# tatsuya-ogawa/metal4-raytracing

Hardware: AMD Instinct MI355X
Metric: Grays/sec (closest-hit + shadow rays traced) at 1920x1080x4spp, dragon; ms/frame (higher is better)
Workload: dtype f32; 1 GPU; c3g: glass dragon scene (configs[2]) 1920x1080x4spp, 8 bounces, one frame per step, single GPU, frames submitted back to back (overlapping frames in flight); scene=c3g, triangles=881218, width=1920, height=1080, spp=4, max_bounces=8, pipeline=wavefront, parallelism=tiles1, rays_per_frame=31537269, sort_bins=0, bvh=sah, frames_in_flight=8, animate=False

## Files before the change

### __graft_entry__.py

```python
import importlib
import lzma
import os
import shutil
import subprocess
import sys

ROOT = os.path.dirname(os.path.abspath(__file__))
PKG = "metal4-raytracing_amd"
ASSET_SRC = os.path.join(ROOT, "tests", "golden", "scene_data")
ASSET_FILES = ["plane.obj", "plane.mtl", "plane-back.obj", "plane-back.mtl", "sphere.obj", "sphere.mtl",
               "dragon.mtl", "train.obj", "train.mtl", "treefir.obj", "treefir.mtl", "teapot.obj",
               "coatball/coatball.obj", "coatball/coatball.mtl"]


def build() -> None:
    env = dict(os.environ, PYTORCH_ROCM_ARCH="gfx950")
    jobs = str(min(16, os.cpu_count() or 1))
    subprocess.run(["make", "-j", jobs, "-C", os.path.join(ROOT, PKG)], check=True, env=env)
    subprocess.run(["make", "-j", jobs, "-C", os.path.join(ROOT, "oracle")], check=True, env=env)
    subprocess.run(["make", "-C", os.path.join(ROOT, "host")], check=True, env=env)
    subprocess.run(["make", "-C", os.path.join(ROOT, "tests", "graph_repro")], check=True, env=env)
    dst = os.path.join(ROOT, "assets")
    for f in ASSET_FILES:
        src, out = os.path.join(ASSET_SRC, f), os.path.join(dst, f)
        if os.path.exists(out):
            continue
        os.makedirs(os.path.dirname(out), exist_ok=True)
        if os.path.exists(src):
            shutil.copyfile(src, out)
        else:
            with lzma.open(src + ".xz", "rb") as fi, open(out + ".tmp", "wb") as fo:
                shutil.copyfileobj(fi, fo)
            os.replace(out + ".tmp", out)
    if ROOT not in sys.path:
        sys.path.insert(0, ROOT)
    rt = importlib.import_module(PKG)
    rt.lib()


def smoke() -> None:
    if ROOT not in sys.path:
        sys.path.insert(0, ROOT)
    import numpy as np
    rt = importlib.import_module(PKG)
    import oracle
    scene = rt.Scene.preset("c1")
    osc = oracle.OracleScene(scene.desc())
    for pipeline in ("wavefront", "megakernel"):
        R = rt.Renderer(scene, 64, 64, device=0, seed=1, pipeline=pipeline)
        R.samplesPerPixel = 1
        R.maxBounces = 2
        u = R.draw()
        g = R.radiance()
        o = osc.render(u, R.random)["radiance"]
        err = np.linalg.norm((g - o)[..., :3], axis=-1) / np.maximum(np.linalg.norm(o[..., :3], axis=-1), 1e-6)
        assert float(err.max()) <= 1e-4, f"smoke parity failed ({pipeline}): max rel L2 {err.max()}"
        print(f"smoke ok ({pipeline}): {rt.version()}, 64x64 c1 frame, max rel L2 {err.max():.3g}, "
              f"bitwise {np.mean(np.all(g[..., :3] == o[..., :3], axis=-1)):.4f}")
        R.close()

if __name__ == "__main__":
    build()
    if len(sys.argv) > 1 and sys.argv[1] == "smoke":
        smoke()
```

### metal4-raytracing_amd/csrc/rt_device.h

```cpp
#pragma once
#include <hip/hip_runtime.h>
#include "rt_math.h"
#include "../../include/rt_types.h"
#include "rt_bvh.h"

namespace rt {

constexpr int kStackSize = 16;
constexpr int kBlock = 256;

struct RootBoxes;
struct DevScene {
    const float* tris;
    const Bvh8Node* nodes8;
    const RootBoxes* root_box;
    const uint4* tri_info;
    const float4* pos;
    const float4* prev_pos;
    const float4* nrm;
    const float4* tri_nrm;
    const float* inst;
    const float* prev_inst;
    const Material* materials;
    const Light* lights;
    const HaltonDim* halton;
    const uint16_t* tri_bin;
    int max_submeshes;
    int num_materials;
    int num_tris;
    int num_nodes8;
    const uchar4* tex_texels = nullptr;
    const uint4* tex_info = nullptr;
    const int4* mat_tex = nullptr;
    const float2* uv = nullptr;
    const float* tex_lut = nullptr;
    int textured = 0;
};

struct Hit {
    float t;
    uint32_t id;
    float u, v;
};

__host__ __device__ __forceinline__ f3 ld3(const float4& v) { return mk3(v.x, v.y, v.z); }

constexpr int kTriFloats = 16;
__host__ __device__ __forceinline__ const float* tri_rec(const float* tris, uint32_t slot) {
    return tris + (size_t)kTriFloats * slot;
}
struct Win3 { float a, b, c; };
__host__ __device__ __forceinline__ f3 tri_window(const float* rec, int v, int kz) {
    const Win3 w = *reinterpret_cast<const Win3*>(rec + 5 * v + kz);
    return mk3(w.a, w.b, w.c);
}
__host__ __device__ __forceinline__ uint32_t tri_id_at(const float* tris, uint32_t fidx) {
    return *reinterpret_cast<const uint32_t*>(reinterpret_cast<const char*>(tris) + fidx * 4u + 60u);
}
__host__ __device__ __forceinline__ f3 tri_window_at(const float* tris, uint32_t fidx) {
    const Win3 w = *reinterpret_cast<const Win3*>(reinterpret_cast<const char*>(tris) + fidx * 4u);
    return mk3(w.a, w.b, w.c);
}
__host__ __device__ __forceinline__ uint32_t tri_id(const float* rec) { return __builtin_bit_cast(uint32_t, rec[15]); }
__host__ __device__ __forceinline__ f3 tri_vertex(const float* rec, int v) { return mk3(rec[5 * v], rec[5 * v + 1], rec[5 * v + 2]); }
__host__ __device__ __forceinline__ void tri_store(float* rec, const float* w, uint32_t id) {
    for (int v = 0; v < 3; ++v) {
        rec[5 * v + 0] = w[3 * v + 0];
        rec[5 * v + 1] = w[3 * v + 1];
        rec[5 * v + 2] = w[3 * v + 2];
        rec[5 * v + 3] = w[3 * v + 0];
        rec[5 * v + 4] = w[3 * v + 1];
    }
    rec[15] = __builtin_bit_cast(float, id);
}

__host__ __device__ __forceinline__ f3 xform(const float* m, f3 p, float w) {
    f3 c0 = mk3(m[0], m[1], m[2]), c1 = mk3(m[3], m[4], m[5]), c2 = mk3(m[6], m[7], m[8]), c3 = mk3(m[9], m[10], m[11]);
    return ((c0 * p.x + c1 * p.y) + c2 * p.z) + c3 * w;
}

struct TraceCounters {
    uint32_t nodes;
    uint32_t tris;
    uint32_t lds_nodes;
};

struct RaySetup {
    f3 o;
    RayPre pre;
    float ix, iy, iz;
    float ox, oy, oz;
    uint32_t dneg;
};

__host__ __device__ __forceinline__ RaySetup ray_setup(f3 o, f3 d) {
    RaySetup R;
    R.pre = ray_precompute(d);
    R.o = rot3(o, R.pre.kz);
    auto safe_inv = [](float x) {
        x = fabsf(x) < 1e-30f ? copysignf(1e-30f, x) : x;
#if defined(__HIP_DEVICE_COMPILE__)
        return __builtin_amdgcn_rcpf(x);
#else
        return 1.0f / x;
#endif
    };
    R.ix = safe_inv(d.x);
    R.iy = safe_inv(d.y);
    R.iz = safe_inv(d.z);
    R.ox = o.x * R.ix;
    R.oy = o.y * R.iy;
    R.oz = o.z * R.iz;
    R.dneg = (d.x < 0.0f ? 1u : 0u) | (d.y < 0.0f ? 2u : 0u) | (d.z < 0.0f ? 4u : 0u);
    return R;
}

__host__ __device__ __forceinline__ float byte_f(uint32_t w, int b) { return (float)((w >> (8 * b)) & 0xffu); }

struct NodeU3 { uint32_t x, y, z; };
struct NodeWords {
    float4 h0;
    NodeU3 h1;
    uint4 qx, qy, qz;
};
__host__ __device__ __forceinline__ NodeWords load_node8(const Bvh8Node* nodes, uint32_t ni) {
    const char* base = reinterpret_cast<const char*>(nodes);
    const uint32_t o = ni * (uint32_t)sizeof(Bvh8Node);
    NodeWords w;
    w.h0 = *reinterpret_cast<const float4*>(base + o);
    w.h1 = *reinterpret_cast<const NodeU3*>(base + (o + 16u));
    w.qx = *reinterpret_cast<const uint4*>(base + (o + 32u));
    w.qy = *reinterpret_cast<const uint4*>(base + (o + 48u));
    w.qz = *reinterpret_cast<const uint4*>(base + (o + 64u));
    return w;
}

__host__ __device__ __forceinline__ uint32_t spread_nibbles(uint32_t x) {
    x = (x | (x << 12)) & 0x000F000Fu;
    x = (x | (x << 6)) & 0x03030303u;
    x = (x | (x << 3)) & 0x11111111u;
    return x * 15u;
}
__host__ __device__ __forceinline__ uint32_t tri_slot(uint32_t tri_base, uint32_t tri_valid, int k) {
    return tri_base + (uint32_t)__builtin_popcount(tri_valid & ((1u << k) - 1u));
}

__host__ __device__ __forceinline__ uint32_t node8_hit_slots(const NodeWords& W, const RaySetup& R, float tmin, float tmax) {
    const float4 h0 = W.h0;
    const uint4 qx = W.qx, qy = W.qy, qz = W.qz;
    const uint32_t ew = __builtin_bit_cast(uint32_t, h0.w);
    const float sx = __builtin_bit_cast(float, (ew & 0xffu) << 23);
    const float sy = __builtin_bit_cast(float, ((ew >> 8) & 0xffu) << 23);
    const float sz = __builtin_bit_cast(float, ((ew >> 16) & 0xffu) << 23);
    const float ax = sx * R.ix, ay = sy * R.iy, az = sz * R.iz;
    const float bx = __builtin_fmaf(h0.x, R.ix, -R.ox);
    const float by = __builtin_fmaf(h0.y, R.iy, -R.oy);
    const float bz = __builtin_fmaf(h0.z, R.iz, -R.oz);
    const uint32_t nx0 = R.ix >= 0.0f ? qx.x : qx.z, nx1 = R.ix >= 0.0f ? qx.y : qx.w;
    const uint32_t fx0 = R.ix >= 0.0f ? qx.z : qx.x, fx1 = R.ix >= 0.0f ? qx.w : qx.y;
    const uint32_t ny0 = R.iy >= 0.0f ? qy.x : qy.z, ny1 = R.iy >= 0.0f ? qy.y : qy.w;
    const uint32_t fy0 = R.iy >= 0.0f ? qy.z : qy.x, fy1 = R.iy >= 0.0f ? qy.w : qy.y;
    const uint32_t nz0 = R.iz >= 0.0f ? qz.x : qz.z, nz1 = R.iz >= 0.0f ? qz.y : qz.w;
    const uint32_t fz0 = R.iz >= 0.0f ? qz.z : qz.x, fz1 = R.iz >= 0.0f ? qz.w : qz.y;
    const float tf_max = tmax * 1.0000004f;
    uint32_t hm = 0;
    #pragma unroll
    for (int c = 0; c < 8; ++c) {
        const int b = c & 3;
        const uint32_t wnx = c < 4 ? nx0 : nx1, wfx = c < 4 ? fx0 : fx1;
        const uint32_t wny = c < 4 ? ny0 : ny1, wfy = c < 4 ? fy0 : fy1;
        const uint32_t wnz = c < 4 ? nz0 : nz1, wfz = c < 4 ? fz0 : fz1;
        const float tnx = __builtin_fmaf(byte_f(wnx, b), ax, bx), tfx = __builtin_fmaf(byte_f(wfx, b), ax, bx);
        const float tny = __builtin_fmaf(byte_f(wny, b), ay, by), tfy = __builtin_fmaf(byte_f(wfy, b), ay, by);
        const float tnz = __builtin_fmaf(byte_f(wnz, b), az, bz), tfz = __builtin_fmaf(byte_f(wfz, b), az, bz);
        const float tn = fmaxf(fmaxf(tnx, tny), fmaxf(tnz, tmin));
        const float tf = fminf(fminf(tfx, tfy), fminf(tfz, tf_max));
        const bool hit = tn <= tf;
        hm |= hit ? (1u << c) : 0u;
    }
    return hm;
}
__host__ __device__ __forceinline__ void node8_decode(uint32_t hm, uint32_t ew, const NodeU3& h1, uint32_t dneg,
                                                      uint32_t& ihits, uint32_t& tmask, uint32_t& tvalid,
                                                      uint32_t& child_base, uint32_t& tri_base, bool& flip) {
    const int axis = (int)((ew >> 24) & 3u);
    const uint32_t k_int = ew >> 28;
    ihits = hm & ((1u << k_int) - 1u);
    tmask = spread_nibbles(hm >> k_int) & h1.z;
    tvalid = h1.z;
    child_base = h1.x;
    tri_base = h1.y;
    flip = (dneg >> axis) & 1u;
}
__host__ __device__ __forceinline__ void test_node8_words(const NodeWords& W, const RaySetup& R, float tmin, float tmax,
                                                          uint32_t& ihits, uint32_t& tmask, uint32_t& tvalid,
                                                          uint32_t& child_base, uint32_t& tri_base, bool& flip) {
    const uint32_t hm = node8_hit_slots(W, R, tmin, tmax);
    node8_decode(hm, __builtin_bit_cast(uint32_t, W.h0.w), W.h1, R.dneg, ihits, tmask, tvalid, child_base, tri_base, flip);
}

#ifndef RT_ROOT_MASK
#define RT_ROOT_MASK 1
#endif
constexpr uint32_t kRootValid = 0x100u;
__host__ __device__ __forceinline__ uint32_t root_word(const NodeWords& root, f3 o, f3 d, float tmax) {
#if RT_ROOT_MASK
    return kRootValid | node8_hit_slots(root, ray_setup(o, d), 0.0f, tmax);
#else
    return 0u;
#endif
}
#ifndef RT_ROOT_TIGHT
#define RT_ROOT_TIGHT 1
#endif
struct RootBoxes {
    float b[3][2][8];
    uint32_t used;
    uint32_t reserved[3];
};
static_assert(sizeof(RootBoxes) == 208, "RootBoxes: 48 planes and the used word, 16-B rows");

__host__ __device__ __forceinline__ bool root_child_bounds(const Bvh8Node* nodes, const float* node_box, const float* tris,
                                                           int c, float lo[3], float hi[3]) {
    const Bvh8Node& nd = nodes[0];
    for (int a = 0; a < 3; ++a) {
        lo[a] = INFINITY;
        hi[a] = -INFINITY;
    }
    if (nd.q[c] == 255 && nd.q[8 + c] == 0) return false;
    const int k_int = nd.axis_k >> 4;
    if (c < k_int) {
        const float* bx = node_box + 6 * (size_t)(nd.child_base + (uint32_t)c);
        for (int a = 0; a < 3; ++a) {
            lo[a] = bx[a];
            hi[a] = bx[3 + a];
        }
    } else {
        const int j = c - k_int;
        const uint32_t first = nd.tri_base + bvh8_leaf_first(nd.tri_valid, j), n = bvh8_leaf_count(nd.tri_valid, j);
        for (uint32_t t = 0; t < n; ++t)
            for (int q = 0; q < 3; ++q) {
                const f3 v = tri_vertex(tri_rec(tris, first + t), q);
                lo[0] = fminf(lo[0], v.x); hi[0] = fmaxf(hi[0], v.x);
                lo[1] = fminf(lo[1], v.y); hi[1] = fmaxf(hi[1], v.y);
                lo[2] = fminf(lo[2], v.z); hi[2] = fmaxf(hi[2], v.z);
            }
        if (n == 0) return false;
    }
    return true;
}
constexpr float kRootPadRel = 1.0f / 524288.0f;
__host__ __device__ __forceinline__ void root_box_store(RootBoxes& B, int c, bool used, const float lo[3], const float hi[3],
                                                        const float pad[3]) {
    for (int a = 0; a < 3; ++a) {
        B.b[a][0][c] = used ? lo[a] - pad[a] : INFINITY;
        B.b[a][1][c] = used ? hi[a] + pad[a] : -INFINITY;
    }
}
__host__ __device__ inline void root_boxes_fill(RootBoxes& B, const Bvh8Node* nodes, const float* node_box, const float* tris) {
    float lo[8][3], hi[8][3], m[3] = {0.0f, 0.0f, 0.0f};
    bool used[8];
    for (int c = 0; c < 8; ++c) {
        used[c] = root_child_bounds(nodes, node_box, tris, c, lo[c], hi[c]);
        for (int a = 0; a < 3; ++a)
            if (used[c]) m[a] = fmaxf(m[a], fmaxf(fabsf(lo[c][a]), fabsf(hi[c][a])));
    }
    const float pad[3] = {kRootPadRel * m[0], kRootPadRel * m[1], kRootPadRel * m[2]};
    B.used = 0u;
// ... 106 lines not shown
```

### metal4-raytracing_amd/csrc/rt_math.h

```cpp
#pragma once

#include <stdint.h>
#include <math.h>

#if defined(__HIPCC__) || defined(__HIP_DEVICE_COMPILE__)
#include <hip/hip_runtime.h>
#define RT_HD __host__ __device__ __forceinline__
#else
#define RT_HD static inline
#endif

#if defined(__clang__)
#pragma clang fp contract(off)
#endif

namespace rt {

struct f3 { float x, y, z; };
struct f2 { float x, y; };

RT_HD f3 mk3(float x, float y, float z) { f3 r; r.x = x; r.y = y; r.z = z; return r; }
RT_HD f3 operator+(f3 a, f3 b) { return mk3(a.x + b.x, a.y + b.y, a.z + b.z); }
RT_HD f3 operator-(f3 a, f3 b) { return mk3(a.x - b.x, a.y - b.y, a.z - b.z); }
RT_HD f3 operator-(f3 a) { return mk3(-a.x, -a.y, -a.z); }
RT_HD f3 operator*(f3 a, f3 b) { return mk3(a.x * b.x, a.y * b.y, a.z * b.z); }
RT_HD f3 operator*(f3 a, float s) { return mk3(a.x * s, a.y * s, a.z * s); }
RT_HD f3 operator*(float s, f3 a) { return mk3(s * a.x, s * a.y, s * a.z); }
RT_HD f3 operator/(f3 a, float s) { return mk3(a.x / s, a.y / s, a.z / s); }
RT_HD float dot(f3 a, f3 b) { return (a.x * b.x + a.y * b.y) + a.z * b.z; }
RT_HD f3 cross(f3 a, f3 b) {
    return mk3(a.y * b.z - a.z * b.y, a.z * b.x - a.x * b.z, a.x * b.y - a.y * b.x);
}
RT_HD float length(f3 a) { return sqrtf(dot(a, a)); }
RT_HD bool length_lt_1e10(f3 a) { return dot(a, a) < 0x1.79ca1p-67f; }
RT_HD bool length_lt_1e3(f3 a) { return dot(a, a) < 0x1.0c6f7ap-20f; }
RT_HD bool length_gt_1e4(f3 a) { return dot(a, a) > 0x1.5798eep-27f; }
RT_HD f3 normalize(f3 a) { float inv = 1.0f / sqrtf(dot(a, a)); return a * inv; }
RT_HD float clampf(float x, float lo, float hi) { return fminf(fmaxf(x, lo), hi); }
RT_HD float saturate(float x) { return clampf(x, 0.0f, 1.0f); }
RT_HD float mixf(float x, float y, float a) { return x + (y - x) * a; }
RT_HD f3 mix3(f3 x, f3 y, float a) { return mk3(mixf(x.x, y.x, a), mixf(x.y, y.y, a), mixf(x.z, y.z, a)); }
RT_HD f3 mix3v(f3 x, f3 y, f3 a) { return mk3(mixf(x.x, y.x, a.x), mixf(x.y, y.y, a.y), mixf(x.z, y.z, a.z)); }

static constexpr float RT_PI = 3.14159265358979323846f;

RT_HD void sincos_pinned(float x, float* s, float* c) {
    float j = rintf(x * 0.63661977236758134f);
    int q = (int)j;
    float r = x - j * 1.5703125f;
    r = r - j * 4.837512969970703125e-4f;
    r = r - j * 7.54978995489188216e-8f;
    float z = r * r;
    float sr = r + r * z * (-1.6666654611e-1f + z * (8.3321608736e-3f + z * (-1.9515295891e-4f)));
    float cr = (1.0f - 0.5f * z) + z * z * (4.166664568298827e-2f + z * (-1.388731625493765e-3f + z * 2.443315711809948e-5f));
    switch (q & 3) {
        case 0: *s = sr; *c = cr; break;
        case 1: *s = cr; *c = -sr; break;
        case 2: *s = -sr; *c = -cr; break;
        default: *s = -cr; *c = sr; break;
    }
}
RT_HD float cos_pinned(float x) { float s, c; sincos_pinned(x, &s, &c); return c; }
RT_HD float pow5(float x) { float x2 = x * x; return (x2 * x2) * x; }

static constexpr int RT_HALTON_DIMS = 1024;
static constexpr int RT_MAX_BOUNCES = 12;

struct HaltonDim { uint32_t b; uint32_t m; uint32_t sh; float invB; };

inline void halton_table_fill(HaltonDim* t, int n) {
    int have = 0;
    for (uint32_t c = 2; have < n; ++c) {
        bool prime = true;
        for (int k = 0; k < have; ++k) {
            if (t[k].b * t[k].b > c) break;
            if (c % t[k].b == 0) { prime = false; break; }
        }
        if (!prime) continue;
        HaltonDim h;
        h.b = c;
        uint32_t l = 0;
        while ((1u << l) < c) ++l;
        h.m = (uint32_t)(((1ull << (31 + l)) + c - 1) / c);
        h.sh = l - 1;
        h.invB = 1.0f / (float)c;
        t[have++] = h;
    }
}

RT_HD uint32_t umulhi32(uint32_t a, uint32_t b) {
#if defined(__HIP_DEVICE_COMPILE__)
    return __umulhi(a, b);
#else
    return (uint32_t)(((uint64_t)a * (uint64_t)b) >> 32);
#endif
}

RT_HD float halton_fast(int i, const HaltonDim& h) {
    float f = 1.0f, r = 0.0f;
    uint32_t n = (uint32_t)i;
    if (i <= 0) return 0.0f;
    while (n > 0) {
        f = f * h.invB;
        uint32_t q = umulhi32(n, h.m) >> h.sh;
        r = r + f * (float)(n - q * h.b);
        n = q;
    }
    return r;
}

RT_HD uint32_t bitrev32(uint32_t x) {
#if defined(__HIP_DEVICE_COMPILE__)
    return __builtin_bitreverse32(x);
#else
    x = ((x >> 1) & 0x55555555u) | ((x & 0x55555555u) << 1);
    x = ((x >> 2) & 0x33333333u) | ((x & 0x33333333u) << 2);
    x = ((x >> 4) & 0x0f0f0f0fu) | ((x & 0x0f0f0f0fu) << 4);
    x = ((x >> 8) & 0x00ff00ffu) | ((x & 0x00ff00ffu) << 8);
    return (x >> 16) | (x << 16);
#endif
}
RT_HD float halton_base2(int i) {
    if (i <= 0) return 0.0f;
    const uint32_t b = bitrev32((uint32_t)i);
    uint32_t r = b;
    const int drop = 8 - __builtin_clz(b);
    if (drop > 0) {
        const uint32_t half = (b >> (drop - 1)) & 1u, last = (b >> drop) & 1u;
        r = b & ~((1u << drop) - 1u);
        if (half & last) {
            r += 1u << drop;
            if (r == 0u) return 1.0f;
        }
    }
    return (float)r * 2.3283064365386963e-10f;
}

RT_HD f3 sampleCosineWeightedHemisphere(float ux, float uy) {
    float phi = 2.0f * RT_PI * ux;
    float sin_phi, cos_phi;
    sincos_pinned(phi, &sin_phi, &cos_phi);
    float cos_theta = sqrtf(uy);
    float sin_theta = sqrtf(1.0f - cos_theta * cos_theta);
    return mk3(sin_theta * cos_phi, cos_theta, sin_theta * sin_phi);
}
RT_HD f3 alignHemisphereWithNormal(f3 s, f3 normal) {
    f3 up = normal;
    f3 right = normalize(cross(normal, mk3(0.0072f, 1.0f, 0.0034f)));
    f3 forward = cross(right, up);
    return (s.x * right + s.y * up) + s.z * forward;
}
RT_HD float distributionGGX(float NdotH, float alpha) {
    float a2 = alpha * alpha;
    float denom = (NdotH * NdotH) * (a2 - 1.0f) + 1.0f;
    return a2 / fmaxf(RT_PI * denom * denom, 1e-7f);
}
RT_HD float geometrySchlickGGX(float NdotV, float k) {
    return NdotV / fmaxf(NdotV * (1.0f - k) + k, 1e-7f);
}
RT_HD float geometrySmith(float NdotV, float NdotL, float k) {
    return geometrySchlickGGX(NdotV, k) * geometrySchlickGGX(NdotL, k);
}
RT_HD f3 fresnelSchlick(float cosTheta, f3 F0) {
    float p = pow5(clampf(1.0f - cosTheta, 0.0f, 1.0f));
    return mk3(F0.x + (1.0f - F0.x) * p, F0.y + (1.0f - F0.y) * p, F0.z + (1.0f - F0.z) * p);
}

struct RayPre {
    int kz;
    float Sx, Sy, Sz;
};
RT_HD float comp(f3 v, int k) { return k == 0 ? v.x : (k == 1 ? v.y : v.z); }
RT_HD f3 rot3(f3 v, int kz) { return kz == 0 ? mk3(v.x, v.y, v.z) : (kz == 1 ? mk3(v.y, v.z, v.x) : mk3(v.z, v.x, v.y)); }
RT_HD RayPre ray_precompute(f3 d) {
    RayPre p;
    float ax = fabsf(d.x), ay = fabsf(d.y), az = fabsf(d.z);
    int kz = (ax > ay) ? ((ax > az) ? 0 : 2) : ((ay > az) ? 1 : 2);
    const f3 r = rot3(d, kz);
    p.kz = kz;
    p.Sx = r.y / r.x;
    p.Sy = r.z / r.x;
    p.Sz = 1.0f / r.x;
    return p;
}
RT_HD bool intersect_rot(const RayPre& p, f3 o, f3 a, f3 b, f3 c, float tmin, float tmax,
                         float* t_out, float* V_out, float* W_out, float* det_out) {
    const float Akz = a.x - o.x, Bkz = b.x - o.x, Ckz = c.x - o.x;
    const float Ax = (a.y - o.y) - p.Sx * Akz;
    const float Ay = (a.z - o.z) - p.Sy * Akz;
    const float Bx = (b.y - o.y) - p.Sx * Bkz;
    const float By = (b.z - o.z) - p.Sy * Bkz;
    const float Cx = (c.y - o.y) - p.Sx * Ckz;
    const float Cy = (c.z - o.z) - p.Sy * Ckz;
    float U = Cx * By - Cy * Bx;
    float V = Ax * Cy - Ay * Cx;
    float W = Bx * Ay - By * Ax;
    if ((U < 0.0f || V < 0.0f || W < 0.0f) && (U > 0.0f || V > 0.0f || W > 0.0f)) return false;
    float det = (U + V) + W;
    if (det == 0.0f) return false;
    float Az = p.Sz * Akz, Bz = p.Sz * Bkz, Cz = p.Sz * Ckz;
    float T = (U * Az + V * Bz) + W * Cz;
    float t = T / det;
    if (!(t >= tmin && t <= tmax)) return false;
    *t_out = t;
    *V_out = V;
    *W_out = W;
    *det_out = det;
    return true;
}
RT_HD bool intersect_triangle_vw(const RayPre& p, f3 o, f3 v0, f3 v1, f3 v2, float tmin, float tmax,
                                 float* t_out, float* V_out, float* W_out, float* det_out) {
    return intersect_rot(p, rot3(o, p.kz), rot3(v0, p.kz), rot3(v1, p.kz), rot3(v2, p.kz), tmin, tmax, t_out, V_out,
                         W_out, det_out);
}

}
```

### metal4-raytracing_amd/csrc/rt_trav.h

```cpp
#pragma once
#include "rt_device.h"

namespace rt {

struct Trav {
    RaySetup R;
    float best, bu, bv, bdet;
    uint32_t best_id, g_base, g_hits, t_base, t_mask, t_valid;
    bool g_flip, hit_any;
    int sp;
};

__host__ __device__ __forceinline__ void trav_start(Trav& T, f3 o, f3 d, float tmax) {
    T.R = ray_setup(o, d);
    T.best = tmax;
    T.best_id = 0xffffffffu;
    T.bu = T.bv = 0.0f;
    T.bdet = 1.0f;
    T.g_base = 0;
    T.g_hits = 1;
    T.g_flip = false;
    T.t_mask = 0;
    T.sp = 0;
    T.hit_any = false;
}

__host__ __device__ __forceinline__ bool trav_start_root(Trav& T, f3 o, f3 d, float tmax, uint32_t word, const RootHead& H) {
    trav_start(T, o, d, tmax);
    if (!(word & kRootValid)) return false;
    node8_decode(word & 0xffu, H.ew, H.h1, T.R.dneg, T.g_hits, T.t_mask, T.t_valid, T.g_base, T.t_base, T.g_flip);
    return true;
}

__host__ __device__ __forceinline__ uint32_t next_node(Trav& T, int* stack, bool& overflow) {
    if (!T.g_hits) {
        --T.sp;
        const uint32_t ent = (uint32_t)stack[T.sp * kBlock];
        unpack_group(ent, T.g_base, T.g_flip, T.g_hits);
    }
    const int r = T.g_flip ? highest_bit(T.g_hits) : lowest_bit(T.g_hits);
    T.g_hits &= ~(1u << r);
    if (T.g_hits) {
        if (T.sp < kStackSize) {
            stack[T.sp * kBlock] = (int)pack_group(T.g_base, T.g_flip, T.g_hits);
            ++T.sp;
        } else {
            overflow = true;
        }
    }
    return T.g_base + (uint32_t)r;
}

template <bool COUNT>
__host__ __device__ __forceinline__ void node_step(const DevScene& S, Trav& T, int* stack, TraceCounters& tc, bool& overflow,
                                                   float cull) {
    const uint32_t ni = next_node(T, stack, overflow);
    if (COUNT) tc.nodes++;
    const NodeWords w = load_node8(S.nodes8, ni);
    test_node8_words(w, T.R, 0.0f, fminf(cull, T.best), T.g_hits, T.t_mask, T.t_valid, T.g_base, T.t_base, T.g_flip);
}

template <bool COUNT>
__host__ __device__ __forceinline__ bool trav_step(const DevScene& S, Trav& T, bool any, int* stack, TraceCounters& tc,
                                                   bool& overflow, float cull) {
    bool tdone = false;
    if (T.t_mask != 0u) {
        const int k0 = lowest_bit(T.t_mask);
        T.t_mask &= T.t_mask - 1u;
        const bool two = T.t_mask != 0u;
        const int k1 = two ? lowest_bit(T.t_mask) : k0;
        if (two) T.t_mask &= T.t_mask - 1u;
        const uint32_t kz = (uint32_t)T.R.pre.kz;
        const uint32_t f0 = tri_slot(T.t_base, T.t_valid, k0) * (uint32_t)kTriFloats + kz;
        const uint32_t f1 = tri_slot(T.t_base, T.t_valid, k1) * (uint32_t)kTriFloats + kz;
        const f3 a0 = tri_window_at(S.tris, f0), a1 = tri_window_at(S.tris, f0 + 5u), a2 = tri_window_at(S.tris, f0 + 10u);
        const uint32_t ida = tri_id_at(S.tris, f0 - kz);
        const f3 b0 = tri_window_at(S.tris, f1), b1 = tri_window_at(S.tris, f1 + 5u), b2 = tri_window_at(S.tris, f1 + 10u);
        const uint32_t idb = tri_id_at(S.tris, f1 - kz);
        if (COUNT) tc.tris += two ? 2u : 1u;
        auto accept = [&](float t, float u, float v, float dt, uint32_t id) {
            if (any) {
                T.hit_any = true;
                tdone = true;
            } else if (t < T.best || id < T.best_id) {
                T.best = t;
                T.best_id = id;
                T.bu = u;
                T.bdet = dt;
                T.bv = v;
            }
        };
        float t, u, v, dt;
        if (intersect_rot(T.R.pre, T.R.o, a0, a1, a2, 0.0f, fminf(cull, T.best), &t, &u, &v, &dt)) accept(t, u, v, dt, ida);
        if (two && !tdone && intersect_rot(T.R.pre, T.R.o, b0, b1, b2, 0.0f, fminf(cull, T.best), &t, &u, &v, &dt))
            accept(t, u, v, dt, idb);
    }
    if (!tdone && T.t_mask == 0u && (T.g_hits != 0u || T.sp > 0)) node_step<COUNT>(S, T, stack, tc, overflow, cull);
    return tdone || (T.t_mask == 0u && T.g_hits == 0u && T.sp == 0);
}

}
```

### metal4-raytracing_amd/csrc/rt_wavefront.hip

```cpp
#include "rt_shade.h"
#include "rt_trav.h"
#include "rt_wavefront.h"
#include "rt_wf_queue.h"

#include <array>
#include <utility>

namespace rt {

namespace {

constexpr uint32_t kNoKey = 0xffffffffu;

__device__ __forceinline__ void ts_start(const WfParams& Q, int ts) {
    if (ts >= 0 && blockIdx.x == 0 && threadIdx.x == 0) Q.W.tstamp[ts * kTsStride] = __builtin_amdgcn_s_memrealtime();
}
__device__ __forceinline__ void ts_end(const WfParams& Q, int ts, uint32_t* done) {
    if (ts < 0 || lane_id() != 0) return;
    if (atomicAdd(done, 1u) == (blockDim.x + 63u) / 64u - 1u)
        atomicMax(&Q.W.tstamp[ts * kTsStride + kTsLine * (1 + (int)(blockIdx.x % (uint32_t)kTsXcds))],
                  (unsigned long long)__builtin_amdgcn_s_memrealtime());
}

__device__ __forceinline__ void stat_add(const WfParams& Q, int word, uint32_t v) {
// ... 285 lines not shown
            h.id = __float_as_uint(hv.y);
            h.u = hv.z;
            h.v = hv.w;
            pid = __float_as_uint(o.w);
            if (!SORTED || h.id != 0xffffffffu) {
                uint4 meta;
                PathRegs p;
                load_path(P, Q, o, d, [&]() { return SORTED ? Q.W.sorted[ce] : ld_stream(&Q.W.qc[cur][ce]); }, FULL, pid,
                          meta, p);
                const f3 a = p.accum;
                int sample = (int)meta.y;
                rayO = ld3(o);
                rayD = ld3(d);
                shade_step<FULL, false>(S, U, halton, (int)meta.w, sample, rayO, rayD, h, p, sample == 0 && p.step == 0,
                                 zero2, false, zero2, r);
                write_pixel_outputs(P, meta.x, r, h, FULL);
                nstate = pack_state(p.bounce, p.tpass, p.step);
                front = likely_long(p);
                ncol = make_float4(p.color.x, p.color.y, p.color.z, __uint_as_float(meta.w));
                if (__float_as_uint(p.accum.x) != __float_as_uint(a.x) || __float_as_uint(p.accum.y) != __float_as_uint(a.y) ||
                    __float_as_uint(p.accum.z) != __float_as_uint(a.z)) {
                    if (!FULL) {
                        const float4 s = Q.W.p_accum[pid];
                        p.accum = mk3(s.x + p.accum.x, s.y + p.accum.y, s.z + p.accum.z);
                    }
                    Q.W.p_accum[pid] = make_float4(p.accum.x, p.accum.y, p.accum.z, 0.0f);
                }
            }
        }
        const uint32_t rwn = r.next ? producer_root_word(lds_root, rayO, rayD, INFINITY) : 0u;
        const bool dead = r.next && root_retires(rwn);
        n_retired += (uint32_t)__popcll(__ballot(dead));
        r.next = r.next && !dead;
        const bool pr[3] = {r.shadow, r.next && front, r.next && !front};
        uint32_t* const ctr[3] = {&Q.W.counts[cslot(kCntShadowQ + shard)], &Q.W.counts[cslot(next * kShards + shard)],
                                  &Q.W.counts[cslot(kCntBack + next * kShards + shard)]};
        uint32_t slots[3];
        const uint32_t oct = (rayD.x < 0.0f ? 1u : 0u) | (rayD.y < 0.0f ? 2u : 0u) | (rayD.z < 0.0f ? 4u : 0u);
        block_alloc3_oct(pr, oct, ctr, bao, slots);
        const uint32_t ns = slots[0], nr = front ? slots[1] : Q.seg_cap - 1u - slots[2];
        if (r.shadow) {
            sqout[3 * (size_t)ns] = make_float4(r.so.x, r.so.y, r.so.z, __uint_as_float(pid));
            sqout[3 * (size_t)ns + 1] = make_float4(r.sd.x, r.sd.y, r.sd.z, r.stmax);
            sqout[3 * (size_t)ns + 2] = make_float4(r.contrib.x, r.contrib.y, r.contrib.z,
                                                    __uint_as_float(producer_root_word(lds_root, r.so, r.sd, r.stmax)));
        }
        if (r.next) {
            qout[2 * (size_t)nr] = make_float4(rayO.x, rayO.y, rayO.z, __uint_as_float(pid));
            qout[2 * (size_t)nr + 1] = make_float4(rayD.x, rayD.y, rayD.z, __uint_as_float(nstate));
            qcout[nr] = ncol;
            qrout[nr] = rwn;
        }
    }
    flush_producer(P, Q, n_retired, 0);
}

__device__ __forceinline__ void sort_range(uint32_t n, uint32_t& beg, uint32_t& end) {
    beg = (uint32_t)(((uint64_t)n * blockIdx.x) / kSortBlocks);
    end = (uint32_t)(((uint64_t)n * (blockIdx.x + 1)) / kSortBlocks);
}

__device__ __forceinline__ uint32_t sort_key(const DevScene& S, const WfParams& Q, uint32_t e, uint32_t shift) {
    const uint32_t id = __float_as_uint(Q.W.hits[e].y);
    return id == 0xffffffffu ? kNoKey : ((uint32_t)S.tri_bin[id] >> shift);
}

__global__ void __launch_bounds__(kSortThreads) wf_sort_hist(DevScene S, WfParams Q, int cur) {
    __shared__ uint32_t h[kSortMaxBins];
    if (tail_mode(Q)) return;
    const uint32_t shift = __builtin_ctz(kSortMaxBins) - __builtin_ctz(Q.sort_bins);
    const uint32_t K = Q.sort_bins;
    const QueueShards qs = load_queue(Q.W.counts, cur, Q.seg_cap);
    for (uint32_t k = threadIdx.x; k < K; k += kSortThreads) h[k] = 0;
    __syncthreads();
    uint32_t beg, end;
    sort_range(queue_len(qs), beg, end);
    for (uint32_t g = beg + threadIdx.x; g < end; g += kSortThreads) {
        const uint32_t k = sort_key(S, Q, dense_entry(qs, g, Q.seg_cap), shift);
        if (k != kNoKey) atomicAdd(&h[k], 1u);
    }
    __syncthreads();
    for (uint32_t k = threadIdx.x; k < K; k += kSortThreads) Q.W.sort_table[(size_t)k * kSortBlocks + blockIdx.x] = h[k];
}

__global__ void __launch_bounds__(kSortBlocks) wf_sort_rowscan(WfParams Q) {
    __shared__ uint32_t w[kSortBlocks / 64];
    if (tail_mode(Q)) return;
    uint32_t* row = Q.W.sort_table + (size_t)blockIdx.x * kSortBlocks;
    const uint32_t v = row[threadIdx.x];
    const uint32_t incl = wave_incl_scan(v);
    uint32_t base, total;
    block_prefix<kSortBlocks / 64>(lane_id() == 63, incl, w, base, total);
    row[threadIdx.x] = base + incl - v;
    if (threadIdx.x == kSortBlocks - 1) Q.W.sort_total[blockIdx.x] = total;
}

__global__ void __launch_bounds__(kSortThreads) wf_sort_scatter(DevScene S, WfParams Q, int cur) {
    __shared__ uint32_t off[kSortMaxBins];
    if (tail_mode(Q)) return;
    const uint32_t shift = __builtin_ctz(kSortMaxBins) - __builtin_ctz(Q.sort_bins);
    __shared__ uint32_t w[kSortThreads / 64];
    const uint32_t K = Q.sort_bins, per = K / kSortThreads;
    const QueueShards qs = load_queue(Q.W.counts, cur, Q.seg_cap);
    uint32_t loc[kSortMaxBins / kSortThreads];
    uint32_t s = 0;
    for (uint32_t i = 0; i < per; ++i) {
        loc[i] = s;
        s += Q.W.sort_total[threadIdx.x * per + i];
    }
    const uint32_t incl = wave_incl_scan(s);
    uint32_t base, total;
    block_prefix<kSortThreads / 64>(lane_id() == 63, incl, w, base, total);
    const uint32_t excl = base + incl - s;
    for (uint32_t i = 0; i < per; ++i) {
        const uint32_t k = threadIdx.x * per + i;
        off[k] = excl + loc[i] + Q.W.sort_table[(size_t)k * kSortBlocks + blockIdx.x];
    }
    if (blockIdx.x == 0 && threadIdx.x == kSortThreads - 1) Q.W.counts[cslot(kCntSorted)] = total;
    __syncthreads();
    const float4* qin = Q.W.q[cur];
    uint32_t beg, end;
    sort_range(queue_len(qs), beg, end);
    for (uint32_t g = beg + threadIdx.x; g < end; g += kSortThreads) {
        const uint32_t e = dense_entry(qs, g, Q.seg_cap);
        const float4 hv = Q.W.hits[e];
        const uint32_t id = __float_as_uint(hv.y);
        if (id == 0xffffffffu) continue;
        const uint32_t pos = atomicAdd(&off[(uint32_t)S.tri_bin[id] >> shift], 1u);
        const float4 o = qin[2 * (size_t)e], d = qin[2 * (size_t)e + 1];
        Q.W.sorted[4 * (size_t)pos] = o;
        Q.W.sorted[4 * (size_t)pos + 1] = d;
        Q.W.sorted[4 * (size_t)pos + 2] = hv;
        if (__float_as_uint(d.w) != 0u) Q.W.sorted[4 * (size_t)pos + 3] = Q.W.qc[cur][e];
    }
}

__device__ __forceinline__ void connect_flush(const WfParams& Q, const float4* qin, uint32_t* pend, uint32_t& npend) {
    __builtin_amdgcn_fence(__ATOMIC_SEQ_CST, "wavefront");
    __builtin_amdgcn_wave_barrier();
    const uint32_t lane = lane_id();
    if (lane < npend) {
        const uint32_t e = pend[lane];
        const float4 o4 = qin[3 * (size_t)e];
        const float4 c = qin[3 * (size_t)e + 2];
        const uint32_t pid = __float_as_uint(o4.w);
        const float4 a = Q.W.p_accum[pid];
        Q.W.p_accum[pid] = make_float4(a.x + c.x, a.y + c.y, a.z + c.z, 0.0f);
    }
    __builtin_amdgcn_fence(__ATOMIC_SEQ_CST, "wavefront");
    __builtin_amdgcn_wave_barrier();
    npend = 0;
}

template <bool ANY, bool COUNT>
#ifndef RT_EXTEND_WAVES
#define RT_EXTEND_WAVES 8
#endif
__global__ void __launch_bounds__(kBlock) __attribute__((amdgpu_waves_per_eu(ANY ? 8 : RT_EXTEND_WAVES, ANY ? 8 : RT_EXTEND_WAVES)))
wf_trace(DevScene S, const FrameParams* __restrict__ Pp, WfParams Q, int cur, int ts) {
    const FrameParams& P = *Pp;
    __shared__ int lds_stack[kStackSize * kBlock];
    int* stack = &lds_stack[threadIdx.x];
    if (Q.dev_ctl) {
        const bool tm = tail_mode(Q);
        if (ANY) {
            if (tm) return;
        } else {
            if (tm || queue_len(load_queue(Q.W.counts, cur, Q.seg_cap)) < Q.tail) {
                if (!tm && blockIdx.x == 0 && threadIdx.x == 0) {
                    Q.W.counts[cslot(kCntTailMode)] = 1u;
                    Q.W.counts[cslot(kCntFinishQ)] = (uint32_t)cur;
                }
                return;
            }
        }
    }
    __shared__ uint32_t ts_done;
    if (threadIdx.x == 0) ts_done = 0u;
    ts_start(Q, ts);
    __syncthreads();
    const uint32_t n = ANY ? load_prefix(Q.W.counts + cslot(kCntShadowQ)).end[kShards - 1]
                           : queue_len(load_queue(Q.W.counts, cur, Q.seg_cap));
    if (Q.dev_ctl) {
        stat_add(Q, kStatTraceRays, n);
        stat_add(Q, kStatTraceLaunches, 1u);
        if (!ANY) {
            stat_add(Q, kStatRounds, 1u);
            stat_add(Q, kStatExtendRays, n);
        }
    }
    if (!ANY && blockIdx.x == 0 && threadIdx.x < 3 * kShards) {
        const int next = 1 - cur;
        const uint32_t k = threadIdx.x & (kShards - 1), part = threadIdx.x / kShards;
        Q.W.counts[cslot(part == 0 ? next * kShards + k : part == 1 ? kCntShadowQ + k : kCntBack + next * kShards + k)] = 0;
    }
    if (blockIdx.x == 0 && threadIdx.x < kShards)
        Q.W.counts[cslot((ANY ? kCntChunkExtend : kCntChunkConnect) + threadIdx.x)] = 0;
    const float4* qin = ANY ? Q.W.sq : Q.W.q[cur];
    const int qstride = ANY ? 3 : 2;
    const RootHead root = load_root_head(S);
    const uint32_t xcd = blockIdx.x & 7u;
    uint32_t* const chunk_ctr = Q.W.counts + cslot((ANY ? kCntChunkConnect : kCntChunkExtend) + (int)xcd);
    uint32_t xl, xend;
    if (ANY) {
        xl = xend = min(__builtin_amdgcn_readfirstlane(Q.W.counts[cslot(kCntShadowQ + (int)xcd)]), Q.seg_cap);
    } else {
        xl = min(__builtin_amdgcn_readfirstlane(Q.W.counts[cslot(cur * kShards + (int)xcd)]), Q.seg_cap);
        xend = xl + min(__builtin_amdgcn_readfirstlane(Q.W.counts[cslot(kCntBack + cur * kShards + (int)xcd)]),
                        Q.seg_cap - xl);
    }
    const uint32_t xbeg = 0, ebase = xcd * Q.seg_cap;
    uint32_t wnext = 0, wend = 0;
    bool exhausted = false;

    TraceCounters tc{0, 0, 0};
    bool overflow = false;
    uint32_t rays = 0;
    bool active = false;
    uint32_t e = 0;
    Trav T;
    trav_start(T, mk3(0, 0, 0), mk3(1, 0, 0), 0.0f);
    uint32_t steps = 0;
    __shared__ uint32_t lds_pend_all[ANY ? kBlock : 1];
    uint32_t* const lds_pend = &lds_pend_all[ANY ? (threadIdx.x & ~63u) : 0u];
    uint32_t npend = 0;

    while (true) {
        const unsigned long long idle = __ballot(!active);
        const bool refill = __popcll(idle) >= Q.refill_min || idle == ~0ull;
        if (wnext >= wend && !exhausted && refill) {
            uint32_t base = 0;
            if (lane_id() == 0) base = atomicAdd(chunk_ctr, (uint32_t)Q.chunk);
            base = xbeg + __builtin_amdgcn_readfirstlane(base);
            if (base >= xend) {
                exhausted = true;
            } else {
                wnext = base;
                wend = min(base + (uint32_t)Q.chunk, xend);
            }
        }
        if (idle != 0ull && wnext < wend && refill) {
            if (!active) {
                uint32_t g = wnext + mbcnt64(idle);
                if (g < wend) {
                    e = ebase + (ANY ? g : seg_pos(g, xl, Q.seg_cap));
                    float4 o4 = qin[(size_t)qstride * e];
                    float4 d4 = qin[(size_t)qstride * e + 1];
                    const uint32_t rw = ANY ? reinterpret_cast<const uint32_t*>(&qin[(size_t)qstride * e + 2])[3] : Q.W.qr[cur][e];
                    if (trav_start_root(T, ld3(o4), ld3(d4), ANY ? d4.w : INFINITY, rw, root) && COUNT) tc.nodes++;
                    active = true;
                    rays++;
                    if (COUNT) steps = 0;
                }
            }
            wnext += (uint32_t)__popcll(idle);
        }
        if (__ballot(active) == 0ull) {
            if (ANY) connect_flush(Q, qin, lds_pend, npend);
            break;
        }
        bool acc = false;
        if (active) {
            if (COUNT) ++steps;
            if (trav_step<COUNT>(S, T, ANY, stack, tc, overflow, T.best)) {
                active = false;
                if (COUNT && Q.diag) {
                    atomicAdd(&Q.W.counts[kWfDiagSteps + (ANY ? kDiagStepBins : 0) + (31 - __builtin_clz(steps))], 1u);
                    atomicMax(&Q.W.counts[kWfDiagSteps + 2 * kDiagStepBins + (ANY ? 1 : 0)], steps);
                }
                if (ANY) acc = !T.hit_any;
                else Q.W.hits[e] = make_float4(T.best, __uint_as_float(T.best_id), T.bu / T.bdet, T.bv / T.bdet);
            }
        }
        if (ANY) {
            const unsigned long long m = __ballot(acc);
            if (m != 0ull) {
                const uint32_t k = (uint32_t)__popcll(m);
                if (npend + k > 64u) connect_flush(Q, qin, lds_pend, npend);
                if (acc) lds_pend[npend + mbcnt64(m)] = e;
                npend += k;
            }
        }
    }
    ts_end(Q, ts, &ts_done);
    flush_counters(P, ANY ? 0 : rays, ANY ? rays : 0, 0, tc, COUNT, overflow, true);
}

template <bool COUNT, bool FULL, bool TEAM>
__global__ void __launch_bounds__(kBlock) __attribute__((amdgpu_waves_per_eu(4, 4)))
wf_finish_step(DevScene S, const FrameParams* __restrict__ Pp, WfParams Q, int cur, int ts) {
    const FrameParams& P = *Pp;
    if (cur < 0) cur = (int)__builtin_amdgcn_readfirstlane(Q.W.counts[cslot(kCntFinishQ)]);
    __shared__ int lds_stack[kStackSize * kBlock];
    __shared__ HaltonDim lds_halton[kHaltonLds];
    __shared__ MatRec lds_mat[kMatLds];
    __shared__ float4 lds_inst[3 * kInstLds];
    __shared__ Light lds_light[kLightLds];
    __shared__ float lds_sray[6][kBlock];
    __shared__ float lds_tx[4][kBlock];
    int* stack = &lds_stack[threadIdx.x];
    __shared__ uint32_t ts_done;
    if (threadIdx.x == 0) ts_done = 0u;
    ts_start(Q, ts);
    const ShadeTabs halton = load_tabs(S, lds_halton, lds_mat, lds_inst, lds_light, P.U.lightCount);
    const Uniforms& U = P.U;
    const QueueShards qs = load_queue(Q.W.counts, cur, Q.seg_cap);
    const uint32_t n = queue_len(qs);
    if (Q.dev_ctl) stat_add(Q, kStatFinish, 1u);
    if (Q.dev_ctl && n > 0) stat_add(Q, kStatRounds, 1u);
    const float4* qin = Q.W.q[cur];
    const uint32_t kChunk = (uint32_t)Q.fchunk;
    constexpr int kIdle = 0, kClosest = 1, kShadow = 2, kReady = 3;
    TraceCounters tc{0, 0, 0};
    bool overflow = false;
    uint32_t n_closest = 0, n_shadow = 0;
    f2 zero2;
    zero2.x = 0.0f;
    zero2.y = 0.0f;
    uint32_t wnext = 0, wend = 0;
    bool exhausted = false;
    int mode = kIdle;
    uint32_t pid = 0;
    uint4 meta = make_uint4(0, 0, 0, 0);
    PathRegs p;
    p.color = p.accum = mk3(0, 0, 0);
    p.bounce = p.tpass = p.step = 0;
    f3 rayO = mk3(0, 0, 0), rayD = mk3(0, 0, 0), contrib = mk3(0, 0, 0);
    bool next = false;
    Trav T;
    trav_start(T, mk3(0, 0, 0), mk3(1, 0, 0), 0.0f);
    uint32_t segs = 0, max_segs = 0, iters = 0;
    const uint64_t t_start = Q.diag ? __builtin_amdgcn_s_memrealtime() : 0;
    __shared__ uint32_t diag_x[kBlock / 64][3];
#define RT_DX diag_x[__builtin_amdgcn_readfirstlane(threadIdx.x) / 64u]
    if (Q.diag && lane_id() == 0) RT_DX[0] = RT_DX[1] = RT_DX[2] = 0xffffffffu;
    uint64_t t_shade = 0;
    uint32_t n_pass = 0, n_shaded = 0;
    auto end_path = [&]() {
        Q.W.p_accum[pid] = make_float4(p.accum.x, p.accum.y, p.accum.z, 0.0f);
        if (Q.diag > 1) {
            const uint32_t b0 = min(meta.z & 0xffu, (uint32_t)kDiagLenBounces - 1u), tp0 = (meta.z >> 8) & 0xffu;
            atomicAdd(&Q.W.counts[kWfDiagLen + ((tp0 ? (uint32_t)kDiagLenBounces : 0u) + b0) * (uint32_t)kDiagLenBins +
                                  min(segs, (uint32_t)kDiagLenBins - 1u)], 1u);
        }
        mode = kIdle;
        max_segs = max(max_segs, segs);
        segs = 0;
    };

    auto shade_hit = [&](StepResult& r) {
        Hit h;
        h.t = T.best;
        h.id = T.best_id;
        h.u = T.bu / T.bdet;
        h.v = T.bv / T.bdet;
        const int sample = (int)meta.y;
        shade_step<FULL, false>(S, U, halton, (int)meta.w, sample, rayO, rayD, h, p, sample == 0 && p.step == 0, zero2,
                                false, zero2, r);
        write_pixel_outputs(P, meta.x, r, h, FULL);
        next = r.next;
    };
    auto sray_store = [&](f3 o, f3 d) {
        lds_sray[0][threadIdx.x] = o.x;
        lds_sray[1][threadIdx.x] = o.y;
        lds_sray[2][threadIdx.x] = o.z;
        lds_sray[3][threadIdx.x] = d.x;
        lds_sray[4][threadIdx.x] = d.y;
        lds_sray[5][threadIdx.x] = d.z;
    };
    auto sray_load = [&](uint32_t slot, f3& o, f3& d) {
        o = mk3(lds_sray[0][slot], lds_sray[1][slot], lds_sray[2][slot]);
        d = mk3(lds_sray[3][slot], lds_sray[4][slot], lds_sray[5][slot]);
    };

    struct StepAt {
        bool start_next;
        bool in_regs;
        bool fresh;
    };
    constexpr StepAt kInLoop = {true, true, false}, kBeforeDrain = {false, true, false}, kInDrain = {false, false, true};
    bool fresh = false;
    auto next_query = [&](const StepAt at) {
        if (at.start_next) trav_start(T, rayO, rayD, INFINITY);
        mode = kClosest;
        n_closest++;
        segs++;
        if (at.fresh) fresh = true;
    };
    auto query_ended = [&](const StepAt at, bool any, bool occluded) {
        if (any) {
            if (!occluded)
                p.accum = p.accum + (at.in_regs ? contrib
                                                : mk3(lds_tx[1][threadIdx.x], lds_tx[2][threadIdx.x], lds_tx[3][threadIdx.x]));
            if (next) next_query(at);
            else end_path();
        } else if (T.best_id == 0xffffffffu) {
            end_path();
        } else {
            mode = kReady;
        }
    };
    auto path_step = [&](const StepAt at) {
        StepResult r;
        shade_hit(r);
        if (r.shadow) {
            if (at.in_regs) {
                contrib = r.contrib;
                trav_start(T, r.so, r.sd, r.stmax);
            } else {
// ... 394 lines not shown
```

Before: 11.54 Grays/s.

## Precompute ray direction setup per 64-ray chunk in LDS before refill

During ray refill in wf_trace, the kernel now computes the shear constants (Sx, Sy, Sz) for the next 64 queued rays cooperatively, one ray per lane, and stores them in per-wave LDS. Idle lanes then read their precomputed values, so the division-heavy setup runs across the whole wave instead of only on the lanes being refilled. The refill window is capped at the prepared chunk. In exchange it adds extra LDS, wave barriers, a second direction load per ray, and recomputes kz and a select-based rotation on each lane. A non-default build variant keeps the old path.

```diff
diff --git a/__graft_entry__.py b/__graft_entry__.py
--- a/__graft_entry__.py
+++ b/__graft_entry__.py
@@ -16,7 +16,7 @@
 def build() -> None:
     env = dict(os.environ, PYTORCH_ROCM_ARCH="gfx950")
     jobs = str(min(16, os.cpu_count() or 1))
-    subprocess.run(["make", "-j", jobs, "-C", os.path.join(ROOT, PKG)], check=True, env=env)
+    subprocess.run(["make", "-j", jobs, "-C", os.path.join(ROOT, PKG), "all", "chunk_prep_off"], check=True, env=env)
     subprocess.run(["make", "-j", jobs, "-C", os.path.join(ROOT, "oracle")], check=True, env=env)
     subprocess.run(["make", "-C", os.path.join(ROOT, "host")], check=True, env=env)
     subprocess.run(["make", "-C", os.path.join(ROOT, "tests", "graph_repro")], check=True, env=env)
diff --git a/metal4-raytracing_amd/csrc/rt_device.h b/metal4-raytracing_amd/csrc/rt_device.h
--- a/metal4-raytracing_amd/csrc/rt_device.h
+++ b/metal4-raytracing_amd/csrc/rt_device.h
@@ -93,10 +93,12 @@
     uint32_t dneg;
 };
 
-__host__ __device__ __forceinline__ RaySetup ray_setup(f3 o, f3 d) {
+__host__ __device__ __forceinline__ RayPre ray_setup_dir(f3 d) { return ray_precompute(d); }
+template <bool SEL = false>
+__host__ __device__ __forceinline__ RaySetup ray_setup_lane(f3 o, f3 d, const RayPre& pre) {
     RaySetup R;
-    R.pre = ray_precompute(d);
-    R.o = rot3(o, R.pre.kz);
+    R.pre = pre;
+    R.o = SEL ? rot3_sel(o, pre.kz) : rot3(o, pre.kz);
     auto safe_inv = [](float x) {
         x = fabsf(x) < 1e-30f ? copysignf(1e-30f, x) : x;
 #if defined(__HIP_DEVICE_COMPILE__)
@@ -114,6 +116,7 @@
     R.dneg = (d.x < 0.0f ? 1u : 0u) | (d.y < 0.0f ? 2u : 0u) | (d.z < 0.0f ? 4u : 0u);
     return R;
 }
+__host__ __device__ __forceinline__ RaySetup ray_setup(f3 o, f3 d) { return ray_setup_lane(o, d, ray_setup_dir(d)); }
 
 __host__ __device__ __forceinline__ float byte_f(uint32_t w, int b) { return (float)((w >> (8 * b)) & 0xffu); }
 
diff --git a/metal4-raytracing_amd/csrc/rt_math.h b/metal4-raytracing_amd/csrc/rt_math.h
--- a/metal4-raytracing_amd/csrc/rt_math.h
+++ b/metal4-raytracing_amd/csrc/rt_math.h
@@ -172,10 +172,16 @@
 };
 RT_HD float comp(f3 v, int k) { return k == 0 ? v.x : (k == 1 ? v.y : v.z); }
 RT_HD f3 rot3(f3 v, int kz) { return kz == 0 ? mk3(v.x, v.y, v.z) : (kz == 1 ? mk3(v.y, v.z, v.x) : mk3(v.z, v.x, v.y)); }
+RT_HD f3 rot3_sel(f3 v, int kz) {
+    return mk3(kz == 0 ? v.x : (kz == 1 ? v.y : v.z), kz == 0 ? v.y : (kz == 1 ? v.z : v.x), kz == 0 ? v.z : (kz == 1 ? v.x : v.y));
+}
+RT_HD int ray_kz(f3 d) {
+    float ax = fabsf(d.x), ay = fabsf(d.y), az = fabsf(d.z);
+    return (ax > ay) ? ((ax > az) ? 0 : 2) : ((ay > az) ? 1 : 2);
+}
 RT_HD RayPre ray_precompute(f3 d) {
     RayPre p;
-    float ax = fabsf(d.x), ay = fabsf(d.y), az = fabsf(d.z);
-    int kz = (ax > ay) ? ((ax > az) ? 0 : 2) : ((ay > az) ? 1 : 2);
+    const int kz = ray_kz(d);
     const f3 r = rot3(d, kz);
     p.kz = kz;
     p.Sx = r.y / r.x;
diff --git a/metal4-raytracing_amd/csrc/rt_trav.h b/metal4-raytracing_amd/csrc/rt_trav.h
--- a/metal4-raytracing_amd/csrc/rt_trav.h
+++ b/metal4-raytracing_amd/csrc/rt_trav.h
@@ -11,8 +11,7 @@
     int sp;
 };
 
-__host__ __device__ __forceinline__ void trav_start(Trav& T, f3 o, f3 d, float tmax) {
-    T.R = ray_setup(o, d);
+__host__ __device__ __forceinline__ void trav_reset(Trav& T, float tmax) {
     T.best = tmax;
     T.best_id = 0xffffffffu;
     T.bu = T.bv = 0.0f;
@@ -24,9 +23,21 @@
     T.sp = 0;
     T.hit_any = false;
 }
+__host__ __device__ __forceinline__ void trav_start(Trav& T, f3 o, f3 d, float tmax) {
+    T.R = ray_setup(o, d);
+    trav_reset(T, tmax);
+}
 
 __host__ __device__ __forceinline__ bool trav_start_root(Trav& T, f3 o, f3 d, float tmax, uint32_t word, const RootHead& H) {
     trav_start(T, o, d, tmax);
+    if (!(word & kRootValid)) return false;
+    node8_decode(word & 0xffu, H.ew, H.h1, T.R.dneg, T.g_hits, T.t_mask, T.t_valid, T.g_base, T.t_base, T.g_flip);
+    return true;
+}
+__host__ __device__ __forceinline__ bool trav_start_root_lane(Trav& T, f3 o, f3 d, float tmax, uint32_t word, const RootHead& H,
+                                                              const RayPre& pre) {
+    T.R = ray_setup_lane<true>(o, d, pre);
+    trav_reset(T, tmax);
     if (!(word & kRootValid)) return false;
     node8_decode(word & 0xffu, H.ew, H.h1, T.R.dneg, T.g_hits, T.t_mask, T.t_valid, T.g_base, T.t_base, T.g_flip);
     return true;
diff --git a/metal4-raytracing_amd/csrc/rt_wavefront.hip b/metal4-raytracing_amd/csrc/rt_wavefront.hip
--- a/metal4-raytracing_amd/csrc/rt_wavefront.hip
+++ b/metal4-raytracing_amd/csrc/rt_wavefront.hip
@@ -461,6 +461,9 @@
     npend = 0;
 }
 
+#ifndef RT_CHUNK_PREP
+#define RT_CHUNK_PREP 1
+#endif
 template <bool ANY, bool COUNT>
 #ifndef RT_EXTEND_WAVES
 #define RT_EXTEND_WAVES 8
@@ -533,6 +536,13 @@
     __shared__ uint32_t lds_pend_all[ANY ? kBlock : 1];
     uint32_t* const lds_pend = &lds_pend_all[ANY ? (threadIdx.x & ~63u) : 0u];
     uint32_t npend = 0;
+#if RT_CHUNK_PREP
+    constexpr int kPrepWords = ANY ? 2 : 3;
+    __shared__ float lds_prep_all[kPrepWords * kBlock];
+    float* const prep = &lds_prep_all[(threadIdx.x & ~63u) * kPrepWords];
+    uint32_t pbase = 0, pend = 0;
+    const uint32_t* const qroot = ANY ? nullptr : Q.W.qr[cur];
+#endif
 
     while (true) {
         const unsigned long long idle = __ballot(!active);
@@ -548,6 +558,47 @@
                 wend = min(base + (uint32_t)Q.chunk, xend);
             }
         }
+#if RT_CHUNK_PREP
+        if (idle != 0ull && wnext < wend && refill) {
+            if (wnext >= pend) {
+                pbase = wnext;
+                pend = min(wnext + 64u, wend);
+                __builtin_amdgcn_fence(__ATOMIC_SEQ_CST, "wavefront");
+                __builtin_amdgcn_wave_barrier();
+                const uint32_t s = lane_id();
+                if (pbase + s < pend) {
+                    const uint32_t pe = ebase + (ANY ? pbase + s : seg_pos(pbase + s, xl, Q.seg_cap));
+                    const RayPre pre = ray_setup_dir(ld3(qin[(size_t)qstride * pe + 1]));
+                    prep[s] = pre.Sx;
+                    prep[64u + s] = pre.Sy;
+                    if (!ANY) prep[(kPrepWords - 1) * 64u + s] = pre.Sz;
+                }
+                __builtin_amdgcn_fence(__ATOMIC_SEQ_CST, "wavefront");
+                __builtin_amdgcn_wave_barrier();
+            }
+            if (!active) {
+                const uint32_t g = wnext + mbcnt64(idle);
+                if (g < pend) {
+                    e = ebase + (ANY ? g : seg_pos(g, xl, Q.seg_cap));
+                    const float4 o4 = qin[(size_t)qstride * e];
+                    const float4 d4 = qin[(size_t)qstride * e + 1];
+                    const uint32_t rw = ANY ? reinterpret_cast<const uint32_t*>(&qin[(size_t)qstride * e + 2])[3] : qroot[e];
+                    const f3 d = ld3(d4);
+                    const uint32_t s = g - pbase;
+                    RayPre pre;
+                    pre.kz = ray_kz(d);
+                    pre.Sx = prep[s];
+                    pre.Sy = prep[64u + s];
+                    pre.Sz = ANY ? 1.0f / rot3_sel(d, pre.kz).x : prep[(kPrepWords - 1) * 64u + s];
+                    if (trav_start_root_lane(T, ld3(o4), d, ANY ? d4.w : INFINITY, rw, root, pre) && COUNT) tc.nodes++;
+                    active = true;
+                    rays++;
+                    if (COUNT) steps = 0;
+                }
+            }
+            wnext = min(wnext + (uint32_t)__popcll(idle), pend);
+        }
+#else
         if (idle != 0ull && wnext < wend && refill) {
             if (!active) {
                 uint32_t g = wnext + mbcnt64(idle);
@@ -564,6 +615,7 @@
             }
             wnext += (uint32_t)__popcll(idle);
         }
+#endif
         if (__ballot(active) == 0ull) {
             if (ANY) connect_flush(Q, qin, lds_pend, npend);
             break;
```

After: 11.62 Grays/s, median of 6. About the same (+0.7%).
